# kahrendt/microWakeWord

Hardware: NVIDIA H100
Metric: streams_x_frames_per_sec (higher is better)
Workload: dtype f32

## Files before the change

### microwakeword_b200/csrc/mww_frontend.cu

```cuda
#include <cuda_runtime.h>
#include <stdlib.h>

#include "mww_frontend_dev.cuh"
#include "mww_kernels.h"

namespace mww {

__device__ __forceinline__ void cp_async16(void *smem_dst, const void *gmem_src) {
    const unsigned dst = (unsigned)__cvta_generic_to_shared(smem_dst);
    asm volatile("cp.async.cg.shared.global [%0], [%1], 16;" ::"r"(dst), "l"(gmem_src));
}
__device__ __forceinline__ void cp_async_commit_and_wait_all() {
    asm volatile("cp.async.commit_group;\ncp.async.wait_group 0;" ::: "memory");
}

__device__ __forceinline__ void k1_load_audio_async(int tid, K1Smem &sm, int buf, const int16_t *carry, int used,
                                                    const int16_t *audio, int n_samples, int f0) {
    const int base = kHop * f0;
    for (int v = tid; v < kGroupSamples / 8; v += kK1Threads) {
        const int vi = base + 8 * v;
        int16_t *dst = &sm.audio[buf][8 * v];
        if (vi < used) cp_async16(dst, carry + vi);
        else if (vi - used < n_samples) cp_async16(dst, audio + (vi - used));
        else *reinterpret_cast<uint4 *>(dst) = make_uint4(0, 0, 0, 0);
    }
}

__device__ __forceinline__ void k1_packed_load_audio_async(int tid, K1Smem &sm, const int16_t *carry, int used, const int16_t *audio,
                                                           long long audio_stride, int n_samples, long long s0, int n_streams, int spc, int fps) {
    const int span8 = (fps + 2) * (kHop / 8), used8 = used / 8, n8 = n_samples / 8;
    int16_t *dst0 = &sm.audio[0][0];
    for (int i = tid; i < spc * span8; i += kK1Threads) {
        const int sl = i / span8, v8 = i - sl * span8;
        int16_t *dst = dst0 + 8 * i;
        const long long s = s0 + sl;
        if (s < n_streams && v8 < used8) cp_async16(dst, carry + s * kWindow + 8 * v8);
        else if (s < n_streams && v8 - used8 < n8) cp_async16(dst, audio + s * audio_stride + 8 * (v8 - used8));
        else *reinterpret_cast<uint4 *>(dst) = make_uint4(0, 0, 0, 0);
    }
}

template <bool kFuseK2, int kOcc>
__global__ void __launch_bounds__(kK1Threads, kOcc)
k1_spectral_kernel(FrontendParams P, const int16_t *__restrict__ carry, int used,
                   const int16_t *__restrict__ audio, long long audio_stride, int n_samples, int n_frames,
                   int groups_per_block, int vec_ok, uint32_t *__restrict__ vout, uint32_t *__restrict__ estimate,
                   uint16_t *__restrict__ feat, long long feat_stream_stride) {
    extern __shared__ __align__(16) unsigned char k1_smem_raw[];
    K1Smem &sm = *reinterpret_cast<K1Smem *>(k1_smem_raw);
    const int tid = threadIdx.x;
    const long long s = blockIdx.x;
    K1Lane lane;
    if (kOcc <= 3) k1_lane_init(tid, P, lane);
    else k1_stage_lane_twiddles(tid, sm, P);
    const K1LaneShared lane_sh{&sm.lane_tw[tid & 15][0]};
    k1_stage_tables(tid, sm, P);

    const int n_groups = (n_frames + kFramesPerGroup - 1) / kFramesPerGroup;
    const int g_begin = blockIdx.y * groups_per_block;
    const int g_end = min(g_begin + groups_per_block, n_groups);
    const int16_t *my_carry = carry + s * kWindow;
    const int16_t *my_audio = audio + s * audio_stride;
    uint32_t est = 0;
    if (kFuseK2 && tid < kNumChannels) est = estimate[s * kNumChannels + tid];
    if (g_begin < g_end) {
        if (vec_ok) k1_load_audio_async(tid, sm, 0, my_carry, used, my_audio, n_samples, g_begin * kFramesPerGroup);
        else k1_load_audio(tid, sm, 0, my_carry, used, my_audio, n_samples, g_begin * kFramesPerGroup);
    }
    for (int g = g_begin; g < g_end; ++g) {
        const int buf = (g - g_begin) & 1;
        cp_async_commit_and_wait_all();
        __syncthreads();
        if (g + 1 < g_end) {
            if (vec_ok) k1_load_audio_async(tid, sm, buf ^ 1, my_carry, used, my_audio, n_samples, (g + 1) * kFramesPerGroup);
            else k1_load_audio(tid, sm, buf ^ 1, my_carry, used, my_audio, n_samples, (g + 1) * kFramesPerGroup);
        }
        const int f0 = g * kFramesPerGroup;
        K1Pass1Ctx ctx;
        k1_window_fft1<2>(tid, sm, buf, (kHop / 2) * (tid >> 4), P, ctx);
        __syncthreads();
        if (kOcc <= 3) k1_fft_pass2(tid, sm, lane); else k1_fft_pass2(tid, sm, lane_sh);
        __syncthreads();
        k1_real_energy(tid, sm, P);
        __syncthreads();
        const int f = f0 + (tid >> 4);
        if (!kFuseK2) {
            k1_filterbank(tid, sm, P, f < n_frames ? vout + (s * n_frames + f) * kNumChannels : nullptr);
        } else {
            k1_filterbank(tid, sm, P, &sm.A[tid >> 4][0]);
            __syncthreads();
            const int n_valid = min(kFramesPerGroup, n_frames - f0);
            if (tid < kNumChannels) k2_group_chain(tid, sm, n_valid, est);
            __syncthreads();
            k2_group_outputs(tid, sm, n_valid, feat + s * feat_stream_stride + (long long)f0 * kNumChannels);
        }
    }
    if (kFuseK2 && tid < kNumChannels) estimate[s * kNumChannels + tid] = est;
}

__global__ void __launch_bounds__(kK1Threads, 3)
k1_spectral_hop_kernel(FrontendParams P, const int16_t *__restrict__ carry, int used, const int16_t *__restrict__ audio,
                       long long audio_stride, int n_samples, int n_frames, int hop, uint32_t *__restrict__ estimate,
                       uint16_t *__restrict__ feat, long long feat_stream_stride) {
    extern __shared__ __align__(16) unsigned char k1_smem_raw[];
    K1Smem &sm = *reinterpret_cast<K1Smem *>(k1_smem_raw);
    const int tid = threadIdx.x;
    const long long s = blockIdx.x;
    K1Lane lane;
    k1_lane_init(tid, P, lane);
    k1_stage_tables(tid, sm, P);
    const int fpg = k1_hop_frames_per_group(hop);
    const int n_groups = (n_frames + fpg - 1) / fpg;
    const int16_t *my_carry = carry + s * kWindow;
    const int16_t *my_audio = audio + s * audio_stride;
    uint32_t est = 0;
    if (tid < kNumChannels) est = estimate[s * kNumChannels + tid];
    for (int g = 0; g < n_groups; ++g) {
        const int f0 = g * fpg;
        __syncthreads();
        k1_hop_load_audio(tid, sm, my_carry, used, my_audio, n_samples, hop * f0, (fpg - 1) * hop + kWindow);
        __syncthreads();
        K1Pass1Ctx ctx;
        k1_window_fft1<2>(tid, sm, 0, k1_hop_pair_base(tid >> 4, hop, fpg), P, ctx);
        __syncthreads();
        k1_fft_pass2(tid, sm, lane);
        __syncthreads();
        k1_real_energy(tid, sm, P);
        __syncthreads();
        k1_filterbank(tid, sm, P, &sm.A[tid >> 4][0]);
        __syncthreads();
        const int n_valid = min(fpg, n_frames - f0);
        if (tid < kNumChannels) k2_group_chain(tid, sm, n_valid, est);
        __syncthreads();
        k2_group_outputs(tid, sm, n_valid, feat + s * feat_stream_stride + (long long)f0 * kNumChannels);
    }
    if (tid < kNumChannels) estimate[s * kNumChannels + tid] = est;
}

__global__ void __launch_bounds__(kK1Threads, 3)
k1_spectral_packed_kernel(FrontendParams P, const int16_t *__restrict__ carry, int used,
                          const int16_t *__restrict__ audio, long long audio_stride, int n_samples, int n_streams, int fps, int spc,
                          int vec_ok, uint32_t *__restrict__ vout) {
    extern __shared__ __align__(16) unsigned char k1_smem_raw[];
    K1Smem &sm = *reinterpret_cast<K1Smem *>(k1_smem_raw);
    const int tid = threadIdx.x;
    const long long s0 = (long long)blockIdx.x * spc;
    K1Lane lane;
    k1_lane_init(tid, P, lane);
    k1_stage_tables(tid, sm, P);
    if (vec_ok) {
        k1_packed_load_audio_async(tid, sm, carry, used, audio, audio_stride, n_samples, s0, n_streams, spc, fps);
        cp_async_commit_and_wait_all();
    } else {
        k1_packed_load_audio(tid, sm, carry, used, audio, audio_stride, n_samples, s0, n_streams, spc, fps);
    }
    __syncthreads();
    const int fl = tid >> 4;
    K1Pass1Ctx ctx;
    k1_window_fft1<2>(tid, sm, 0, k1_packed_pair_base(fl < spc * fps ? fl : 0, fps), P, ctx);
    __syncthreads();
    k1_fft_pass2(tid, sm, lane);
    __syncthreads();
    k1_real_energy(tid, sm, P);
    __syncthreads();
    const long long s = s0 + fl / fps;
    const bool active = fl < spc * fps && s < n_streams;
    k1_filterbank(tid, sm, P, active ? vout + (s * fps + fl % fps) * kNumChannels : nullptr);
}

__global__ void __launch_bounds__(kK1Threads, 3)
k1k2_packed_kernel(FrontendParams P, int16_t *__restrict__ carry, int used, const int16_t *__restrict__ audio,
                   long long audio_stride, int n_samples, int n_streams, int fps, int spc, int vec_ok, uint32_t *__restrict__ estimate,
                   uint16_t *__restrict__ feat, long long feat_stream_stride, int new_used) {
    extern __shared__ __align__(16) unsigned char k1_smem_raw[];
    K1Smem &sm = *reinterpret_cast<K1Smem *>(k1_smem_raw);
    const int tid = threadIdx.x;
    const long long s0 = (long long)blockIdx.x * spc;
    K1Lane lane;
    k1_lane_init(tid, P, lane);
    k1_stage_tables(tid, sm, P);
    if (vec_ok) {
        k1_packed_load_audio_async(tid, sm, carry, used, audio, audio_stride, n_samples, s0, n_streams, spc, fps);
        cp_async_commit_and_wait_all();
    } else {
        k1_packed_load_audio(tid, sm, carry, used, audio, audio_stride, n_samples, s0, n_streams, spc, fps);
    }
    __syncthreads();
    const int fl = tid >> 4;
    K1Pass1Ctx ctx;
    k1_window_fft1<2>(tid, sm, 0, k1_packed_pair_base(fl < spc * fps ? fl : 0, fps), P, ctx);
    __syncthreads();
    k1_fft_pass2(tid, sm, lane);
    __syncthreads();
    k1_real_energy(tid, sm, P);
    __syncthreads();
    k1_filterbank(tid, sm, P, fl < spc * fps ? &sm.A[fl][0] : nullptr);
    __syncthreads();
    for (int t = tid; t < spc * kNumChannels; t += kK1Threads) {
        const int sl = t / kNumChannels, ch = t - sl * kNumChannels;
        const long long s = s0 + sl;
        if (s < n_streams) {
            const uint32_t smoothing = (ch & 1) ? kOddSmoothing : kEvenSmoothing;
            uint32_t est = estimate[s * kNumChannels + ch];
            uint16_t *out = feat + s * feat_stream_stride + ch;
            for (int f = 0; f < fps; ++f) out[(long long)f * kNumChannels] = k2_channel_step(sm.A[sl * fps + f][ch], est, smoothing, sm.gain_lut, sm.log_lut);
            estimate[s * kNumChannels + ch] = est;
        }
    }
    const int span = (fps + 2) * kHop, consumed = fps * kHop;
    const int16_t *staged = &sm.audio[0][0];
    if (vec_ok) {
        for (int i = tid; i < spc * (kWindow / 8); i += kK1Threads) {
            const int sl = i / (kWindow / 8), v8 = i - sl * (kWindow / 8);
            if (s0 + sl >= n_streams) continue;
            uint4 v = make_uint4(0, 0, 0, 0);
            if (8 * v8 < new_used) v = *reinterpret_cast<const uint4 *>(staged + sl * span + consumed + 8 * v8);
            *reinterpret_cast<uint4 *>(carry + (s0 + sl) * kWindow + 8 * v8) = v;
        }
    } else {
        for (int i = tid; i < spc * kWindow; i += kK1Threads) {
            const int sl = i / kWindow, k = i - sl * kWindow;
            if (s0 + sl >= n_streams) continue;
            carry[(s0 + sl) * kWindow + k] = k < new_used ? staged[sl * span + consumed + k] : (int16_t)0;
        }
    }
}

__global__ void __launch_bounds__(256)
k2_temporal_kernel(FrontendParams P, const uint32_t *__restrict__ vin, int n_streams, int n_frames,
                   uint32_t *__restrict__ estimate, uint16_t *__restrict__ feat, long long feat_stream_stride) {
    __shared__ int16_t gain_lut[128];
    __shared__ uint16_t log_lut[132];
    for (int i = threadIdx.x; i < 128; i += blockDim.x) gain_lut[i] = P.gain_lut[i];
    for (int i = threadIdx.x; i < 132; i += blockDim.x) log_lut[i] = P.log_lut[i];
    __syncthreads();
    const long long idx = (long long)blockIdx.x * blockDim.x + threadIdx.x;
    if (idx >= (long long)n_streams * kNumChannels) return;
    const long long s = idx / kNumChannels;
    const int ch = (int)(idx - s * kNumChannels);
    const uint32_t smoothing = (ch & 1) ? kOddSmoothing : kEvenSmoothing;
    uint32_t est = estimate[idx];
    const uint32_t *v = vin + s * (long long)n_frames * kNumChannels + ch;
    uint16_t *out = feat + s * feat_stream_stride + ch;
    int f = 0;
    for (; f + 4 <= n_frames; f += 4) {
        uint32_t x[4];
#pragma unroll
        for (int q = 0; q < 4; ++q) x[q] = __ldcs(v + (long long)(f + q) * kNumChannels);
#pragma unroll
        for (int q = 0; q < 4; ++q) out[(long long)(f + q) * kNumChannels] = k2_channel_step(x[q], est, smoothing, gain_lut, log_lut);
    }
    for (; f < n_frames; ++f) out[(long long)f * kNumChannels] = k2_channel_step(v[(long long)f * kNumChannels], est, smoothing, gain_lut, log_lut);
    estimate[idx] = est;
}

__global__ void __launch_bounds__(128)
carry_update_kernel(int16_t *__restrict__ carry, int used, const int16_t *__restrict__ audio, long long audio_stride,
                    int n_samples, int consumed, int new_used) {
    const long long s = blockIdx.x;
    int16_t *c = carry + s * kWindow;
    const int16_t *a = audio + s * audio_stride;
    int16_t tmp[4];
#pragma unroll
    for (int q = 0; q < 4; ++q) {
        const int i = threadIdx.x + 128 * q;
        int16_t val = 0;
        if (i < new_used) {
            const int vi = consumed + i;
            val = vi < used ? c[vi] : a[vi - used];
        }
        tmp[q] = val;
    }
    __syncthreads();
#pragma unroll
    for (int q = 0; q < 4; ++q) {
        const int i = threadIdx.x + 128 * q;
        if (i < kWindow) c[i] = tmp[q];
    }
}


namespace {
template <typename K>
cudaError_t k1_opt_in(K kernel, bool (&done)[64]) {
    if (!first_launch_on_this_device(done)) return cudaSuccess;
    return cudaFuncSetAttribute(kernel, cudaFuncAttributeMaxDynamicSharedMemorySize, kK1SmemBytes);
}
}

bool frontend_clip_fuses(int n_streams, int n_frames, int sm_count) {
    return n_frames > 8 && (long long)n_streams >= (long long)sm_count * 3 * 4;
}

cudaError_t launch_k1(const FrontendParams &P, const int16_t *carry, int used, const int16_t *audio,
                      long long audio_stride, int n_samples, int n_streams, int n_frames, uint32_t *vout, int sm_count,
                      cudaStream_t st) {
    if (n_frames <= 0 || n_streams <= 0) return cudaSuccess;
    const int vec_ok = (used % 8 == 0) && (n_samples % 8 == 0) && (audio_stride % 8 == 0) &&
                       (reinterpret_cast<uintptr_t>(audio) % 16 == 0) && (reinterpret_cast<uintptr_t>(carry) % 16 == 0);
    if (n_frames <= 8 && n_streams >= 2) {
        static bool done[64] = {};
        cudaError_t e = k1_opt_in(k1_spectral_packed_kernel, done);
        if (e != cudaSuccess) return e;
        const int spc = k1_packed_streams(n_frames);
        const unsigned grid = (unsigned)((n_streams + spc - 1) / spc);
        k1_spectral_packed_kernel<<<grid, kK1Threads, kK1SmemBytes, st>>>(P, carry, used, audio, audio_stride, n_samples, n_streams, n_frames, spc, vec_ok, vout);
        return cudaGetLastError();
    }
    static bool done[64] = {};
    cudaError_t e = k1_opt_in(k1_spectral_kernel<false, 3>, done);
    if (e != cudaSuccess) return e;
    const int n_groups = (n_frames + kFramesPerGroup - 1) / kFramesPerGroup;
    int chunks = 1;
    const long long want = (long long)sm_count * 3 * 4;
    if (n_streams < want) chunks = (int)min((long long)n_groups, (want + n_streams - 1) / n_streams);
    const int gpb = (n_groups + chunks - 1) / chunks;
    chunks = (n_groups + gpb - 1) / gpb;
    dim3 grid((unsigned)n_streams, (unsigned)chunks);
    k1_spectral_kernel<false, 3><<<grid, kK1Threads, kK1SmemBytes, st>>>(P, carry, used, audio, audio_stride, n_samples, n_frames, gpb, vec_ok, vout,
                                                                      nullptr, nullptr, 0);
    return cudaGetLastError();
}

cudaError_t launch_frontend_clip_fused(const FrontendParams &P, const int16_t *carry, int used, const int16_t *audio, long long audio_stride,
                                       int n_samples, int n_streams, int n_frames, uint32_t *estimate, uint16_t *feat, long long feat_stream_stride,
                                       cudaStream_t st) {
    if (n_frames <= 0 || n_streams <= 0) return cudaSuccess;
    static bool done3[64] = {}, done4[64] = {};
    static const int occ = getenv("MWW_K1_OCC") ? atoi(getenv("MWW_K1_OCC")) : 4;
    cudaError_t e = occ == 3 ? k1_opt_in(k1_spectral_kernel<true, 3>, done3) : k1_opt_in(k1_spectral_kernel<true, 4>, done4);
    if (e != cudaSuccess) return e;
    const int vec_ok = (used % 8 == 0) && (n_samples % 8 == 0) && (audio_stride % 8 == 0) &&
                       (reinterpret_cast<uintptr_t>(audio) % 16 == 0) && (reinterpret_cast<uintptr_t>(carry) % 16 == 0);
    const int n_groups = (n_frames + kFramesPerGroup - 1) / kFramesPerGroup;
    dim3 grid((unsigned)n_streams, 1u);
    if (occ == 3)
        k1_spectral_kernel<true, 3><<<grid, kK1Threads, kK1SmemBytes, st>>>(P, carry, used, audio, audio_stride, n_samples, n_frames, n_groups, vec_ok,
                                                                            nullptr, estimate, feat, feat_stream_stride);
    else
        k1_spectral_kernel<true, 4><<<grid, kK1Threads, kK1SmemBytes, st>>>(P, carry, used, audio, audio_stride, n_samples, n_frames, n_groups, vec_ok,
                                                                            nullptr, estimate, feat, feat_stream_stride);
    return cudaGetLastError();
}

cudaError_t launch_frontend_hop(const FrontendParams &P, const int16_t *carry, int used, const int16_t *audio, long long audio_stride,
                                int n_samples, int n_streams, int n_frames, int hop, uint32_t *estimate, uint16_t *feat,
                                long long feat_stream_stride, cudaStream_t st) {
    if (n_frames <= 0 || n_streams <= 0) return cudaSuccess;
    static bool done[64] = {};
    cudaError_t e = k1_opt_in(k1_spectral_hop_kernel, done);
    if (e != cudaSuccess) return e;
    k1_spectral_hop_kernel<<<(unsigned)n_streams, kK1Threads, kK1SmemBytes, st>>>(P, carry, used, audio, audio_stride, n_samples, n_frames, hop,
                                                                                 estimate, feat, feat_stream_stride);
    return cudaGetLastError();
}

bool frontend_fusable(int used, int n_samples, int n_frames) {
    const int new_used = used + n_samples - n_frames * kHop;
    return n_frames >= 1 && n_frames <= 8 && new_used >= 0 && new_used <= 2 * kHop;
}

cudaError_t launch_frontend_fused(const FrontendParams &P, int16_t *carry, int used, const int16_t *audio,
                                  long long audio_stride, int n_samples, int n_streams, int n_frames, uint32_t *estimate, uint16_t *feat,
                                  long long feat_stream_stride, cudaStream_t st) {
    if (n_streams <= 0) return cudaSuccess;
    static bool done[64] = {};
    cudaError_t e = k1_opt_in(k1k2_packed_kernel, done);
    if (e != cudaSuccess) return e;
    const int vec_ok = (used % 8 == 0) && (n_samples % 8 == 0) && (audio_stride % 8 == 0) &&
                       (reinterpret_cast<uintptr_t>(audio) % 16 == 0) && (reinterpret_cast<uintptr_t>(carry) % 16 == 0);
    const int spc = k1_packed_streams(n_frames);
    const unsigned grid = (unsigned)((n_streams + spc - 1) / spc);
    k1k2_packed_kernel<<<grid, kK1Threads, kK1SmemBytes, st>>>(P, carry, used, audio, audio_stride, n_samples, n_streams, n_frames, spc, vec_ok,
                                                    estimate, feat, feat_stream_stride, used + n_samples - n_frames * kHop);
    return cudaGetLastError();
}

cudaError_t launch_k2(const FrontendParams &P, const uint32_t *vin, int n_streams, int n_frames, uint32_t *estimate,
                      uint16_t *feat, long long feat_stream_stride, cudaStream_t st) {
    if (n_frames <= 0 || n_streams <= 0) return cudaSuccess;
    const long long total = (long long)n_streams * kNumChannels;
    const unsigned blocks = (unsigned)((total + 255) / 256);
    k2_temporal_kernel<<<blocks, 256, 0, st>>>(P, vin, n_streams, n_frames, estimate, feat, feat_stream_stride);
    return cudaGetLastError();
}

cudaError_t launch_carry_update(int16_t *carry, int used, const int16_t *audio, long long audio_stride, int n_samples,
                                int n_streams, int consumed, int new_used, cudaStream_t st) {
    if (n_streams <= 0) return cudaSuccess;
    carry_update_kernel<<<(unsigned)n_streams, 128, 0, st>>>(carry, used, audio, audio_stride, n_samples, consumed, new_used);
    return cudaGetLastError();
}

}
```

### microwakeword_b200/csrc/mww_frontend_dev.cuh

```cuda
#pragma once

#include "mww_common.h"
#include "mww_tables.h"

#if !defined(__CUDA_ARCH__)
#include <math.h>
#endif

namespace mww {

constexpr int kFramesPerGroup = 16;
constexpr int kK1Threads = 256;
constexpr int kRowWords = 272;
constexpr int kGroupSamples = (kFramesPerGroup + 2) * kHop;


struct K1Smem {
    uint32_t A[kFramesPerGroup][kRowWords];
    uint32_t B[kFramesPerGroup][kRowWords];
    int16_t audio[2][kGroupSamples];
    uint16_t lane_max[kFramesPerGroup][16];
    int32_t shift[kFramesPerGroup];
    int32_t fb_coef[kFbCoefWords];
    int16_t gain_lut[128];
    uint16_t log_lut[132];
    uint32_t lane_tw[16][15];
};
constexpr int kK1SmemBytes = (int)sizeof(K1Smem);

MWW_HD void k1_stage_tables(int tid, K1Smem &sm, const FrontendParams &P) {
    for (int i = tid; i < kFbCoefWords; i += kK1Threads) sm.fb_coef[i] = P.fb_coef[i];
    for (int i = tid; i < 128; i += kK1Threads) sm.gain_lut[i] = P.gain_lut[i];
    for (int i = tid; i < 132; i += kK1Threads) sm.log_lut[i] = P.log_lut[i];
}

struct K1Lane {
    int32_t t3r[3], t3i[3];
    int32_t t4r[12], t4i[12];
};

struct K1LaneShared { const uint32_t *row; };


MWW_HD int32_t fixdiv4(int32_t x) { return (x * 8191 + 16384) >> 15; }
MWW_HD int32_t fixdiv2(int32_t x) { return (x * 16383 + 16384) >> 15; }

MWW_HD void cmul_q15(int32_t ar, int32_t ai, int32_t wr, int32_t wi, int32_t &mr, int32_t &mi) {
    mr = (ar * wr - ai * wi + 16384) >> 15;
    mi = (ar * wi + ai * wr + 16384) >> 15;
}

MWW_HD void bfly4_core(int32_t &r0, int32_t &i0, int32_t &r1, int32_t &i1, int32_t &r2, int32_t &i2, int32_t &r3, int32_t &i3) {
    const int32_t s5r = r0 - r2, s5i = i0 - i2;
    const int32_t f0r = r0 + r2, f0i = i0 + i2;
    const int32_t s3r = r1 + r3, s3i = i1 + i3;
    const int32_t s4r = r1 - r3, s4i = i1 - i3;
    r2 = f0r - s3r; i2 = f0i - s3i;
    r0 = f0r + s3r; i0 = f0i + s3i;
    r1 = s5r + s4i; i1 = s5i - s4r;
    r3 = s5r - s4i; i3 = s5i + s4r;
}


MWW_HD uint64_t sq32(uint32_t r) { return (uint64_t)r * r; }

MWW_HD uint32_t isqrt64_round(uint64_t x) {
#if defined(__CUDA_ARCH__)
    const float xf = __ull2float_rn(x);
    const float rs = rsqrtf(xf);
    uint32_t r = __float2uint_rz(xf * rs);
    const int64_t d = (int64_t)(x - sq32(r));
    const int64_t r1 = (int64_t)r + (int64_t)__float2int_rd(__ll2float_rn(d) * (0.5f * rs));
#else
    const float xf = (float)x;
    const float rs = x ? 1.0f / sqrtf(xf) : 0.0f;
    const float rf = xf * rs;
    uint32_t r = rf >= 4294967040.0f ? 0xFFFFFFFFu : (uint32_t)rf;
    const int64_t d = (int64_t)(x - sq32(r));
    const int64_t r1 = (int64_t)r + (int64_t)floorf((float)d * (0.5f * rs));
#endif
    r = r1 > 0xFFFFFFFFll ? 0xFFFFFFFFu : (r1 < 0 ? 0u : (uint32_t)r1);
#pragma unroll
    for (int pass = 0; pass < 2; ++pass) r -= (sq32(r) > x) ? 1u : 0u;
    uint64_t rem = x - sq32(r);
#pragma unroll
    for (int pass = 0; pass < 2; ++pass) {
        const bool up = rem > 2ull * r;
        rem -= up ? 2ull * r + 1 : 0ull;
        r += up ? 1u : 0u;
    }
    const uint32_t cap = (x >> 32) == 0 ? 0xFFFFu : 0xFFFFFFFFu;
    r += (rem > r && r < cap) ? 1u : 0u;
    r = r > cap ? cap : r;
    return x == 0 ? 0u : r;
}

MWW_HD uint32_t isqrt64_round_fast(uint64_t x) {
    if (x >> 48) return isqrt64_round(x);
#if defined(__CUDA_ARCH__)
    const uint32_t r = __double2uint_rz(sqrt(__ull2double_rn(x)) + 0.5);
#else
    const uint32_t r = (uint32_t)(sqrt((double)x) + 0.5);
#endif
    const uint32_t cap = (x >> 32) == 0 ? 0xFFFFu : 0xFFFFFFFFu;
    return r > cap ? cap : r;
}


MWW_HD void k1_lane_init(int tid, const FrontendParams &P, K1Lane &L) {
    const int b = tid & 15;
    for (int j = 0; j < 3; ++j) {
        const uint32_t w = P.tw[4 * b * (j + 1)];
        L.t3r[j] = unpack_lo(w); L.t3i[j] = unpack_hi(w);
    }
    for (int j = 0; j < 4; ++j) {
        const int kp = 16 * j + b;
        for (int q = 0; q < 3; ++q) {
            const uint32_t w = P.tw[kp * (q + 1)];
            L.t4r[3 * j + q] = unpack_lo(w); L.t4i[3 * j + q] = unpack_hi(w);
        }
    }
}

MWW_HD void k1_stage_lane_twiddles(int tid, K1Smem &sm, const FrontendParams &P) {
    for (int i = tid; i < 16 * 15; i += kK1Threads) {
        const int b = i / 15, e = i - 15 * b;
        int idx;
        if (e < 3) idx = 4 * b * (e + 1);
        else { const int j = (e - 3) / 3, q = (e - 3) - 3 * j; idx = (16 * j + b) * (q + 1); }
        sm.lane_tw[b][e] = P.tw[idx];
    }
}
MWW_HD void lane_tw3(const K1Lane &L, int q, int32_t &wr, int32_t &wi) { wr = L.t3r[q]; wi = L.t3i[q]; }
MWW_HD void lane_tw4(const K1Lane &L, int i, int32_t &wr, int32_t &wi) { wr = L.t4r[i]; wi = L.t4i[i]; }
MWW_HD void lane_tw3(const K1LaneShared &L, int q, int32_t &wr, int32_t &wi) { const uint32_t w = L.row[q]; wr = unpack_lo(w); wi = unpack_hi(w); }
MWW_HD void lane_tw4(const K1LaneShared &L, int i, int32_t &wr, int32_t &wi) { const uint32_t w = L.row[3 + i]; wr = unpack_lo(w); wi = unpack_hi(w); }

MWW_HD void k1_load_audio(int tid, K1Smem &sm, int buf, const int16_t *carry, int used, const int16_t *audio, int n_samples, int f0) {
    const int base = kHop * f0;
    for (int i = tid; i < kGroupSamples; i += kK1Threads) {
        const int vi = base + i;
        int16_t s = 0;
        if (vi < used) s = carry[vi];
        else if (vi - used < n_samples) s = audio[vi - used];
        sm.audio[buf][i] = s;
    }
}

MWW_HD int k1_hop_frames_per_group(int hop) {
    const int by_span = (2 * kGroupSamples - kWindow) / hop + 1;
    return by_span < kFramesPerGroup ? by_span : kFramesPerGroup;
}
MWW_HD void k1_hop_load_audio(int tid, K1Smem &sm, const int16_t *carry, int used, const int16_t *audio, int n_samples, int base, int span) {
    int16_t *dst = &sm.audio[0][0];
    for (int i = tid; i < span; i += kK1Threads) {
        const int vi = base + i;
        int16_t s = 0;
        if (vi < used) s = carry[vi];
        else if (vi - used < n_samples) s = audio[vi - used];
        dst[i] = s;
    }
}
MWW_HD int k1_hop_pair_base(int fl, int hop, int fpg) { return (hop / 2) * (fl < fpg ? fl : fpg - 1); }

struct K1Pass1Ctx { int32_t xr[16], xi[16]; };

template <int PART>
MWW_HD void k1_window_fft1(int tid, K1Smem &sm, int buf, int pair_base, const FrontendParams &P, K1Pass1Ctx &ctx) {
    const int fl = tid >> 4, a = tid & 15;
    const int c = (a >> 2) + 4 * (a & 3);
    int32_t (&xr)[16] = ctx.xr;
    int32_t (&xi)[16] = ctx.xi;
    if (PART != 1) {
        const uint32_t *pairs = reinterpret_cast<const uint32_t *>(sm.audio[buf]) + pair_base;
        int32_t mx = 0, mn = 0;
#pragma unroll
        for (int b = 0; b < 16; ++b) {
            const int j = (b >> 2) + 4 * (b & 3);
            if (j == 15) { xr[b] = 0; xi[b] = 0; continue; }
            const int p = c + 16 * j;
            const uint32_t sw = pairs[p];
            const uint32_t cw = P.win_pairs[p];
            const int32_t v0 = (unpack_lo(sw) * unpack_lo(cw)) >> 12;
            const int32_t v1 = (unpack_hi(sw) * unpack_hi(cw)) >> 12;
            xr[b] = v0; xi[b] = v1;
            if (j == 7) {
                const int32_t m0 = v0 == -32768 ? 0 : v0, m1 = v1 == -32768 ? 0 : v1;
                mx = max3i(mx, m0, m1); mn = min3i(mn, m0, m1);
            } else {
                mx = max3i(mx, v0, v1); mn = min3i(mn, v0, v1);
            }
        }
        const int32_t m = mx > -mn ? mx : -mn;
        sm.lane_max[fl][a] = (uint16_t)m;
    }
#if defined(__CUDA_ARCH__)
    if (PART == 2) __syncwarp();
#endif
    if (PART == 0) return;
    int32_t mxa = 0;
#pragma unroll
    for (int i = 0; i < 16; ++i) { const int32_t v = sm.lane_max[fl][i]; mxa = v > mxa ? v : mxa; }
    const int shift = 15 - msb32((uint32_t)mxa);
    if (a == 0) sm.shift[fl] = shift;
    const int32_t k4 = 8191 << shift;
#pragma unroll
    for (int g = 0; g < 4; ++g) {
#pragma unroll
        for (int q = 0; q < 4; ++q) {
            const int b = 4 * g + q;
            const int j = (b >> 2) + 4 * (b & 3);
            if (j == 7) {
                xr[b] = fixdiv4(sext16(xr[b] << shift)); xi[b] = fixdiv4(sext16(xi[b] << shift));
            } else {
                xr[b] = (xr[b] * k4 + 16384) >> 15; xi[b] = (xi[b] * k4 + 16384) >> 15;
            }
        }
        bfly4_core(xr[4 * g], xi[4 * g], xr[4 * g + 1], xi[4 * g + 1], xr[4 * g + 2], xi[4 * g + 2], xr[4 * g + 3], xi[4 * g + 3]);
    }
#pragma unroll
    for (int k = 0; k < 4; ++k) {
#pragma unroll
        for (int q = 0; q < 4; ++q) { xr[k + 4 * q] = fixdiv4(xr[k + 4 * q]); xi[k + 4 * q] = fixdiv4(xi[k + 4 * q]); }
        if (k > 0) {
#pragma unroll
            for (int q = 1; q < 4; ++q) {
                int32_t mr, mi;
                cmul_q15(xr[k + 4 * q], xi[k + 4 * q], P.tw2[(k - 1) * 3 + (q - 1)][0], P.tw2[(k - 1) * 3 + (q - 1)][1], mr, mi);
                xr[k + 4 * q] = mr; xi[k + 4 * q] = mi;
            }
        }
        bfly4_core(xr[k], xi[k], xr[k + 4], xi[k + 4], xr[k + 8], xi[k + 8], xr[k + 12], xi[k + 12]);
    }
#pragma unroll
    for (int b = 0; b < 16; ++b) sm.B[fl][17 * a + b] = pack16(xr[b], xi[b]);
}

MWW_HD int k1_packed_streams(int fps) {
    const int by_slots = kFramesPerGroup / fps;
    const int by_smem = (2 * kGroupSamples) / ((fps + 2) * kHop);
    return by_slots < by_smem ? by_slots : by_smem;
}
MWW_HD void k1_packed_load_audio(int tid, K1Smem &sm, const int16_t *carry, int used, const int16_t *audio, long long audio_stride,
                                 int n_samples, long long s0, int n_streams, int spc, int fps) {
    const int span = (fps + 2) * kHop;
    int16_t *dst = &sm.audio[0][0];
    for (int i = tid; i < spc * span; i += kK1Threads) {
        const int sl = i / span, vi = i - sl * span;
        int16_t v = 0;
        if (s0 + sl < n_streams) {
            if (vi < used) v = carry[(s0 + sl) * kWindow + vi];
            else if (vi - used < n_samples) v = audio[(s0 + sl) * audio_stride + (vi - used)];
        }
        dst[i] = v;
    }
}
MWW_HD int k1_packed_pair_base(int fl, int fps) { return (fl / fps) * ((fps + 2) * (kHop / 2)) + (kHop / 2) * (fl % fps); }

template <typename LaneT>
MWW_HD void k1_fft_pass2(int tid, K1Smem &sm, const LaneT &L) {
    const int fl = tid >> 4, b = tid & 15;
    int32_t yr[16], yi[16];
#pragma unroll
    for (int a = 0; a < 16; ++a) {
        const uint32_t w = sm.B[fl][17 * a + b];
        yr[a] = unpack_lo(w); yi[a] = unpack_hi(w);
    }
#pragma unroll
    for (int c = 0; c < 4; ++c) {
#pragma unroll
        for (int q = 0; q < 4; ++q) { yr[4 * c + q] = fixdiv4(yr[4 * c + q]); yi[4 * c + q] = fixdiv4(yi[4 * c + q]); }
#pragma unroll
        for (int q = 1; q < 4; ++q) {
            int32_t mr, mi, wr, wi;
            lane_tw3(L, q - 1, wr, wi);
            cmul_q15(yr[4 * c + q], yi[4 * c + q], wr, wi, mr, mi);
            yr[4 * c + q] = mr; yi[4 * c + q] = mi;
        }
        bfly4_core(yr[4 * c], yi[4 * c], yr[4 * c + 1], yi[4 * c + 1], yr[4 * c + 2], yi[4 * c + 2], yr[4 * c + 3], yi[4 * c + 3]);
    }
#pragma unroll
    for (int j = 0; j < 4; ++j) {
#pragma unroll
        for (int q = 0; q < 4; ++q) { yr[4 * q + j] = fixdiv4(sext16(yr[4 * q + j])); yi[4 * q + j] = fixdiv4(sext16(yi[4 * q + j])); }
#pragma unroll
        for (int q = 1; q < 4; ++q) {
            int32_t mr, mi, wr, wi;
            lane_tw4(L, 3 * j + q - 1, wr, wi);
            cmul_q15(yr[4 * q + j], yi[4 * q + j], wr, wi, mr, mi);
            yr[4 * q + j] = mr; yi[4 * q + j] = mi;
        }
        bfly4_core(yr[j], yi[j], yr[4 + j], yi[4 + j], yr[8 + j], yi[8 + j], yr[12 + j], yi[12 + j]);
    }
#pragma unroll
    for (int a = 0; a < 16; ++a) sm.A[fl][b + 16 * a] = pack16(yr[a], yi[a]);
}

MWW_HD void k1_real_energy(int tid, K1Smem &sm, const FrontendParams &P) {
    const int fl = tid >> 4, l = tid & 15;
    if (l == 0) { sm.B[fl][0] = 0; sm.B[fl][kEnergyOffset] = 0; }
#pragma unroll
    for (int t = 0; t < 8; ++t) {
        const int k = 1 + 16 * t + l;
        const uint32_t wk = sm.A[fl][k];
        const uint32_t wn = sm.A[fl][kNcfft - k];
        const uint32_t ws = P.super_tw[k - 1];
        const int32_t pr = fixdiv2(unpack_lo(wk)), pi = fixdiv2(unpack_hi(wk));
        const int32_t nr = fixdiv2(unpack_lo(wn)), ni = fixdiv2(sext16(-unpack_hi(wn)));
        const int32_t f1r = pr + nr, f1i = pi + ni;
        const int32_t f2r = pr - nr, f2i = pi - ni;
        int32_t tr, ti;
        cmul_q15(f2r, f2i, unpack_lo(ws), unpack_hi(ws), tr, ti);
        tr = sext16(tr); ti = sext16(ti);
        const int32_t ar = sext16((f1r + tr) >> 1), ai = sext16((f1i + ti) >> 1);
        const int32_t br = sext16((f1r - tr) >> 1), bi = sext16((ti - f1i) >> 1);
        sm.B[fl][k + kEnergyOffset] = (uint32_t)(ar * ar) + (uint32_t)(ai * ai);
        sm.B[fl][kNcfft - k + kEnergyOffset] = (uint32_t)(br * br) + (uint32_t)(bi * bi);
    }
}

struct Pair32 { uint32_t x, y; };
MWW_HD Pair32 load_pair(const uint32_t *p) {
#if defined(__CUDA_ARCH__)
    const uint2 v = *reinterpret_cast<const uint2 *>(p);
    return Pair32{v.x, v.y};
#else
    return Pair32{p[0], p[1]};
#endif
}
MWW_HD void k1_filterbank(int tid, K1Smem &sm, const FrontendParams &P, uint32_t *vout_frame ) {
    const int fl = tid >> 4, l = tid & 15;
    const int sh = sm.shift[fl];
#pragma unroll
    for (int s = 0; s < kFbSlots; ++s) {
        if (fb_len(s) == 0) continue;
        const FbSlot slot = P.fb_slots[l * kFbSlots + s];
        int64_t acc = 0;
        const uint32_t *e = &sm.B[fl][slot.word0];
        const uint32_t *cf = reinterpret_cast<const uint32_t *>(&sm.fb_coef[slot.coef_off]);
#pragma unroll
        for (int j = 0; j < fb_len(s) / 2; ++j) {
            const Pair32 ev = load_pair(e + 2 * j), cv = load_pair(cf + 2 * j);
            acc = mad_wide_s32((int32_t)ev.x, (int32_t)cv.x, acc);
            acc = mad_wide_s32((int32_t)ev.y, (int32_t)cv.y, acc);
        }
        if (slot.ch >= 0 && vout_frame) vout_frame[slot.ch] = isqrt64_round_fast((uint64_t)acc) >> sh;
    }
}


MWW_HD int32_t wide_dynamic_function(uint32_t x, const int16_t *lut) {
    if (x <= 2) return lut[x];
    const int interval = msb32(x);
    const int16_t *p = lut + 4 * interval - 6;
    const int32_t frac = (int32_t)(((interval < 11) ? (x << (11 - interval)) : (x >> (interval - 11))) & 0x3FF);
    int32_t r = ((int32_t)p[2] * frac) >> 5;
    r += (int32_t)((uint32_t)(int32_t)p[1] << 5);
    r *= frac;
    r = (r + (1 << 14)) >> 15;
    r += p[0];
    return (int32_t)(int16_t)r;
}

MWW_HD uint32_t pcan_shrink(uint32_t x) {
    if (x < (2u << 12)) return (x * x) >> 20;
    return (x >> 6) - 64u;
}

MWW_HD uint32_t log_scale(uint32_t x, const uint16_t *lut) {
    const uint32_t integer = (uint32_t)msb32(x) - 1;
    int32_t frac = (int32_t)(x - (1u << integer));
    if (integer < 16) frac <<= (16 - integer); else frac >>= (integer - 16);
    const uint32_t seg = (uint32_t)frac >> 9;
    const int32_t c0 = lut[seg], c1 = lut[seg + 1];
    const int32_t rel = ((c1 - c0) * (frac - (int32_t)(seg << 9))) >> 16;
    const uint32_t log2v = (integer << 16) + (uint32_t)(frac + c0 + rel);
    const uint32_t loge = (uint32_t)((45426ull * log2v + 32768u) >> 16);
    return ((loge << kLogScaleShift) + 32768u) >> 16;
}

MWW_HD uint32_t k2_estimate_update(uint32_t v, uint32_t est, uint32_t smoothing) {
    const uint32_t scaled = v << kSmoothingBits;
    return (uint32_t)((((uint64_t)scaled * smoothing) + ((uint64_t)est * ((1u << kNoiseBits) - smoothing))) >> kNoiseBits);
}

MWW_HD uint16_t k2_output(uint32_t v, uint32_t est, const int16_t *gain_lut, const uint16_t *log_lut) {
    const uint32_t scaled = v << kSmoothingBits;
    const uint32_t e = est > scaled ? scaled : est;
    const uint32_t fl = (uint32_t)(((uint64_t)v * kMinSignalRemaining) >> kNoiseBits);
    const uint32_t sub = (scaled - e) >> kSmoothingBits;
    uint32_t sig = sub > fl ? sub : fl;
    const uint32_t gain = (uint32_t)wide_dynamic_function(est, gain_lut);
    const uint32_t snr = (uint32_t)(((uint64_t)sig * gain) >> kPcanSnrShift);
    sig = pcan_shrink(snr);
    sig <<= kLogCorrectionBits;
    sig = sig > 1 ? log_scale(sig, log_lut) : 0;
    return (uint16_t)(sig < 0xFFFFu ? sig : 0xFFFFu);
}

MWW_HD uint16_t k2_channel_step(uint32_t v, uint32_t &est, uint32_t smoothing, const int16_t *gain_lut, const uint16_t *log_lut) {
    est = k2_estimate_update(v, est, smoothing);
    return k2_output(v, est, gain_lut, log_lut);
}

MWW_HD void k2_group_chain(int ch, K1Smem &sm, int n_valid, uint32_t &est) {
    const uint32_t smoothing = (ch & 1) ? kOddSmoothing : kEvenSmoothing;
    for (int f = 0; f < n_valid; ++f) {
        est = k2_estimate_update(sm.A[f][ch], est, smoothing);
        sm.B[f][ch] = est;
    }
}
MWW_HD void k2_group_outputs(int tid, K1Smem &sm, int n_valid, uint16_t *feat_group ) {
    for (int i = tid; i < n_valid * kNumChannels; i += kK1Threads) {
        const int f = i / kNumChannels, ch = i - f * kNumChannels;
        feat_group[i] = k2_output(sm.A[f][ch], sm.B[f][ch], sm.gain_lut, sm.log_lut);
    }
}

}
```

Before: 460.9 million.

## Stage twiddles in padded smem, shuffle-reduce lane max, defer wide isqrt path

```diff
diff --git a/microwakeword_b200/csrc/mww_frontend.cu b/microwakeword_b200/csrc/mww_frontend.cu
--- a/microwakeword_b200/csrc/mww_frontend.cu
+++ b/microwakeword_b200/csrc/mww_frontend.cu
@@ -10,6 +10,10 @@
     const unsigned dst = (unsigned)__cvta_generic_to_shared(smem_dst);
     asm volatile("cp.async.cg.shared.global [%0], [%1], 16;" ::"r"(dst), "l"(gmem_src));
 }
+__device__ __forceinline__ void cp_async16_zfill(void *smem_dst, const void *gmem_src, bool valid) {
+    const unsigned dst = (unsigned)__cvta_generic_to_shared(smem_dst);
+    asm volatile("cp.async.cg.shared.global [%0], [%1], 16, %2;" ::"r"(dst), "l"(gmem_src), "r"(valid ? 16 : 0));
+}
 __device__ __forceinline__ void cp_async_commit_and_wait_all() {
     asm volatile("cp.async.commit_group;\ncp.async.wait_group 0;" ::: "memory");
 }
@@ -17,12 +21,11 @@
 __device__ __forceinline__ void k1_load_audio_async(int tid, K1Smem &sm, int buf, const int16_t *carry, int used,
                                                     const int16_t *audio, int n_samples, int f0) {
     const int base = kHop * f0;
+#pragma unroll 1
     for (int v = tid; v < kGroupSamples / 8; v += kK1Threads) {
         const int vi = base + 8 * v;
-        int16_t *dst = &sm.audio[buf][8 * v];
-        if (vi < used) cp_async16(dst, carry + vi);
-        else if (vi - used < n_samples) cp_async16(dst, audio + (vi - used));
-        else *reinterpret_cast<uint4 *>(dst) = make_uint4(0, 0, 0, 0);
+        const bool from_carry = vi < used, valid = from_carry || vi - used < n_samples;
+        cp_async16_zfill(&sm.audio[buf][8 * v], from_carry || !valid ? carry + (from_carry ? vi : 0) : audio + (vi - used), valid);
     }
 }
 
diff --git a/microwakeword_b200/csrc/mww_frontend_dev.cuh b/microwakeword_b200/csrc/mww_frontend_dev.cuh
--- a/microwakeword_b200/csrc/mww_frontend_dev.cuh
+++ b/microwakeword_b200/csrc/mww_frontend_dev.cuh
@@ -24,7 +24,8 @@
     int32_t fb_coef[kFbCoefWords];
     int16_t gain_lut[128];
     uint16_t log_lut[132];
-    uint32_t lane_tw[16][15];
+    alignas(16) uint32_t lane_tw[16][15 * 4];
+    alignas(16) int32_t super_tw[128][4];
 };
 constexpr int kK1SmemBytes = (int)sizeof(K1Smem);
 
@@ -32,7 +33,12 @@
     for (int i = tid; i < kFbCoefWords; i += kK1Threads) sm.fb_coef[i] = P.fb_coef[i];
     for (int i = tid; i < 128; i += kK1Threads) sm.gain_lut[i] = P.gain_lut[i];
     for (int i = tid; i < 132; i += kK1Threads) sm.log_lut[i] = P.log_lut[i];
-}
+    for (int i = tid; i < 128; i += kK1Threads) {
+        const uint32_t w = P.super_tw[i];
+        sm.super_tw[i][0] = unpack_lo(w); sm.super_tw[i][1] = unpack_hi(w); sm.super_tw[i][2] = -unpack_hi(w); sm.super_tw[i][3] = 0;
+    }
+}
+static_assert(4 * (sizeof(K1Smem) + 1024) <= 228 * 1024, "K1Smem must leave room for 4 CTAs per SM");
 
 struct K1Lane {
     int32_t t3r[3], t3i[3];
@@ -47,6 +53,10 @@
 
 MWW_HD void cmul_q15(int32_t ar, int32_t ai, int32_t wr, int32_t wi, int32_t &mr, int32_t &mi) {
     mr = (ar * wr - ai * wi + 16384) >> 15;
+    mi = (ar * wi + ai * wr + 16384) >> 15;
+}
+MWW_HD void cmul_q15_nw(int32_t ar, int32_t ai, int32_t wr, int32_t wi, int32_t nwi, int32_t &mr, int32_t &mi) {
+    mr = (ar * wr + ai * nwi + 16384) >> 15;
     mi = (ar * wi + ai * wr + 16384) >> 15;
 }
 
@@ -95,16 +105,17 @@
     return x == 0 ? 0u : r;
 }
 
-MWW_HD uint32_t isqrt64_round_fast(uint64_t x) {
-    if (x >> 48) return isqrt64_round(x);
+MWW_HD uint32_t isqrt64_round_fp64(uint64_t x) {
 #if defined(__CUDA_ARCH__)
     const uint32_t r = __double2uint_rz(sqrt(__ull2double_rn(x)) + 0.5);
 #else
-    const uint32_t r = (uint32_t)(sqrt((double)x) + 0.5);
+    const double s = sqrt((double)x) + 0.5;
+    const uint32_t r = s >= 4294967296.0 ? 0xFFFFFFFFu : (uint32_t)s;
 #endif
     const uint32_t cap = (x >> 32) == 0 ? 0xFFFFu : 0xFFFFFFFFu;
     return r > cap ? cap : r;
 }
+MWW_HD uint32_t isqrt64_round_fast(uint64_t x) { return (x >> 48) ? isqrt64_round(x) : isqrt64_round_fp64(x); }
 
 
 MWW_HD void k1_lane_init(int tid, const FrontendParams &P, K1Lane &L) {
@@ -128,13 +139,24 @@
         int idx;
         if (e < 3) idx = 4 * b * (e + 1);
         else { const int j = (e - 3) / 3, q = (e - 3) - 3 * j; idx = (16 * j + b) * (q + 1); }
-        sm.lane_tw[b][e] = P.tw[idx];
-    }
-}
-MWW_HD void lane_tw3(const K1Lane &L, int q, int32_t &wr, int32_t &wi) { wr = L.t3r[q]; wi = L.t3i[q]; }
-MWW_HD void lane_tw4(const K1Lane &L, int i, int32_t &wr, int32_t &wi) { wr = L.t4r[i]; wi = L.t4i[i]; }
-MWW_HD void lane_tw3(const K1LaneShared &L, int q, int32_t &wr, int32_t &wi) { const uint32_t w = L.row[q]; wr = unpack_lo(w); wi = unpack_hi(w); }
-MWW_HD void lane_tw4(const K1LaneShared &L, int i, int32_t &wr, int32_t &wi) { const uint32_t w = L.row[3 + i]; wr = unpack_lo(w); wi = unpack_hi(w); }
+        const uint32_t w = P.tw[idx];
+        uint32_t *q = &sm.lane_tw[b][4 * e];
+        q[0] = (uint32_t)unpack_lo(w); q[1] = (uint32_t)unpack_hi(w); q[2] = (uint32_t)-unpack_hi(w); q[3] = 0;
+    }
+}
+MWW_HD void lane_tw(const K1Lane &L, int e, int32_t &wr, int32_t &wi, int32_t &nwi) {
+    wr = e < 3 ? L.t3r[e] : L.t4r[e - 3]; wi = e < 3 ? L.t3i[e] : L.t4i[e - 3]; nwi = -wi;
+}
+MWW_HD void load_tw(const void *entry, int32_t &wr, int32_t &wi, int32_t &nwi) {
+#if defined(__CUDA_ARCH__)
+    const int4 v = *reinterpret_cast<const int4 *>(entry);
+    wr = v.x; wi = v.y; nwi = v.z;
+#else
+    const int32_t *p = reinterpret_cast<const int32_t *>(entry);
+    wr = p[0]; wi = p[1]; nwi = p[2];
+#endif
+}
+MWW_HD void lane_tw(const K1LaneShared &L, int e, int32_t &wr, int32_t &wi, int32_t &nwi) { load_tw(L.row + 4 * e, wr, wi, nwi); }
 
 MWW_HD void k1_load_audio(int tid, K1Smem &sm, int buf, const int16_t *carry, int used, const int16_t *audio, int n_samples, int f0) {
     const int base = kHop * f0;
@@ -171,6 +193,7 @@
     const int c = (a >> 2) + 4 * (a & 3);
     int32_t (&xr)[16] = ctx.xr;
     int32_t (&xi)[16] = ctx.xi;
+    int32_t m = 0;
     if (PART != 1) {
         const uint32_t *pairs = reinterpret_cast<const uint32_t *>(sm.audio[buf]) + pair_base;
         int32_t mx = 0, mn = 0;
@@ -191,16 +214,19 @@
                 mx = max3i(mx, v0, v1); mn = min3i(mn, v0, v1);
             }
         }
-        const int32_t m = mx > -mn ? mx : -mn;
-        sm.lane_max[fl][a] = (uint16_t)m;
-    }
-#if defined(__CUDA_ARCH__)
-    if (PART == 2) __syncwarp();
-#endif
+        m = mx > -mn ? mx : -mn;
+        if (PART == 0) sm.lane_max[fl][a] = (uint16_t)m;
+    }
     if (PART == 0) return;
     int32_t mxa = 0;
+#if defined(__CUDA_ARCH__)
+    mxa = m;
+#pragma unroll
+    for (int o = 8; o > 0; o >>= 1) { const int32_t v = __shfl_xor_sync(0xFFFFFFFFu, mxa, o); mxa = v > mxa ? v : mxa; }
+#else
 #pragma unroll
     for (int i = 0; i < 16; ++i) { const int32_t v = sm.lane_max[fl][i]; mxa = v > mxa ? v : mxa; }
+#endif
     const int shift = 15 - msb32((uint32_t)mxa);
     if (a == 0) sm.shift[fl] = shift;
     const int32_t k4 = 8191 << shift;
@@ -272,9 +298,9 @@
         for (int q = 0; q < 4; ++q) { yr[4 * c + q] = fixdiv4(yr[4 * c + q]); yi[4 * c + q] = fixdiv4(yi[4 * c + q]); }
 #pragma unroll
         for (int q = 1; q < 4; ++q) {
-            int32_t mr, mi, wr, wi;
-            lane_tw3(L, q - 1, wr, wi);
-            cmul_q15(yr[4 * c + q], yi[4 * c + q], wr, wi, mr, mi);
+            int32_t mr, mi, wr, wi, nwi;
+            lane_tw(L, q - 1, wr, wi, nwi);
+            cmul_q15_nw(yr[4 * c + q], yi[4 * c + q], wr, wi, nwi, mr, mi);
             yr[4 * c + q] = mr; yi[4 * c + q] = mi;
         }
         bfly4_core(yr[4 * c], yi[4 * c], yr[4 * c + 1], yi[4 * c + 1], yr[4 * c + 2], yi[4 * c + 2], yr[4 * c + 3], yi[4 * c + 3]);
@@ -285,9 +311,9 @@
         for (int q = 0; q < 4; ++q) { yr[4 * q + j] = fixdiv4(sext16(yr[4 * q + j])); yi[4 * q + j] = fixdiv4(sext16(yi[4 * q + j])); }
 #pragma unroll
         for (int q = 1; q < 4; ++q) {
-            int32_t mr, mi, wr, wi;
-            lane_tw4(L, 3 * j + q - 1, wr, wi);
-            cmul_q15(yr[4 * q + j], yi[4 * q + j], wr, wi, mr, mi);
+            int32_t mr, mi, wr, wi, nwi;
+            lane_tw(L, 3 + 3 * j + q - 1, wr, wi, nwi);
+            cmul_q15_nw(yr[4 * q + j], yi[4 * q + j], wr, wi, nwi, mr, mi);
             yr[4 * q + j] = mr; yi[4 * q + j] = mi;
         }
         bfly4_core(yr[j], yi[j], yr[4 + j], yi[4 + j], yr[8 + j], yi[8 + j], yr[12 + j], yi[12 + j]);
@@ -296,7 +322,7 @@
     for (int a = 0; a < 16; ++a) sm.A[fl][b + 16 * a] = pack16(yr[a], yi[a]);
 }
 
-MWW_HD void k1_real_energy(int tid, K1Smem &sm, const FrontendParams &P) {
+MWW_HD void k1_real_energy(int tid, K1Smem &sm, const FrontendParams &) {
     const int fl = tid >> 4, l = tid & 15;
     if (l == 0) { sm.B[fl][0] = 0; sm.B[fl][kEnergyOffset] = 0; }
 #pragma unroll
@@ -304,13 +330,14 @@
         const int k = 1 + 16 * t + l;
         const uint32_t wk = sm.A[fl][k];
         const uint32_t wn = sm.A[fl][kNcfft - k];
-        const uint32_t ws = P.super_tw[k - 1];
+        int32_t wr, wi, nwi;
+        load_tw(sm.super_tw[k - 1], wr, wi, nwi);
         const int32_t pr = fixdiv2(unpack_lo(wk)), pi = fixdiv2(unpack_hi(wk));
         const int32_t nr = fixdiv2(unpack_lo(wn)), ni = fixdiv2(sext16(-unpack_hi(wn)));
         const int32_t f1r = pr + nr, f1i = pi + ni;
         const int32_t f2r = pr - nr, f2i = pi - ni;
         int32_t tr, ti;
-        cmul_q15(f2r, f2i, unpack_lo(ws), unpack_hi(ws), tr, ti);
+        cmul_q15_nw(f2r, f2i, wr, wi, nwi, tr, ti);
         tr = sext16(tr); ti = sext16(ti);
         const int32_t ar = sext16((f1r + tr) >> 1), ai = sext16((f1i + ti) >> 1);
         const int32_t br = sext16((f1r - tr) >> 1), bi = sext16((ti - f1i) >> 1);
@@ -328,23 +355,40 @@
     return Pair32{p[0], p[1]};
 #endif
 }
+MWW_HD uint64_t fb_accumulate(const uint32_t *e, const uint32_t *cf, int len ) {
+    int64_t acc = 0;
+#pragma unroll
+    for (int j = 0; j < len / 2; ++j) {
+        const Pair32 ev = load_pair(e + 2 * j), cv = load_pair(cf + 2 * j);
+        acc = mad_wide_s32((int32_t)ev.x, (int32_t)cv.x, acc);
+        acc = mad_wide_s32((int32_t)ev.y, (int32_t)cv.y, acc);
+    }
+    return (uint64_t)acc;
+}
 MWW_HD void k1_filterbank(int tid, K1Smem &sm, const FrontendParams &P, uint32_t *vout_frame ) {
     const int fl = tid >> 4, l = tid & 15;
     const int sh = sm.shift[fl];
+    bool wide = false;
 #pragma unroll
     for (int s = 0; s < kFbSlots; ++s) {
         if (fb_len(s) == 0) continue;
         const FbSlot slot = P.fb_slots[l * kFbSlots + s];
-        int64_t acc = 0;
-        const uint32_t *e = &sm.B[fl][slot.word0];
-        const uint32_t *cf = reinterpret_cast<const uint32_t *>(&sm.fb_coef[slot.coef_off]);
-#pragma unroll
-        for (int j = 0; j < fb_len(s) / 2; ++j) {
-            const Pair32 ev = load_pair(e + 2 * j), cv = load_pair(cf + 2 * j);
-            acc = mad_wide_s32((int32_t)ev.x, (int32_t)cv.x, acc);
-            acc = mad_wide_s32((int32_t)ev.y, (int32_t)cv.y, acc);
-        }
-        if (slot.ch >= 0 && vout_frame) vout_frame[slot.ch] = isqrt64_round_fast((uint64_t)acc) >> sh;
+        const uint64_t x = fb_accumulate(&sm.B[fl][slot.word0], reinterpret_cast<const uint32_t *>(&sm.fb_coef[slot.coef_off]), fb_len(s));
+        wide |= (x >> 48) != 0;
+        if (slot.ch >= 0 && vout_frame) vout_frame[slot.ch] = isqrt64_round_fp64(x) >> sh;
+    }
+    if (wide && vout_frame) {
+#pragma unroll 1
+        for (int s = 0; s < kFbSlots; ++s) {
+            const FbSlot slot = P.fb_slots[l * kFbSlots + s];
+            if (fb_len(s) == 0 || slot.ch < 0) continue;
+            const uint32_t *e = &sm.B[fl][slot.word0];
+            const int32_t *cf = &sm.fb_coef[slot.coef_off];
+            int64_t acc = 0;
+#pragma unroll 1
+            for (int j = 0; j < fb_len(s); ++j) acc = mad_wide_s32((int32_t)e[j], cf[j], acc);
+            if ((uint64_t)acc >> 48) vout_frame[slot.ch] = isqrt64_round((uint64_t)acc) >> sh;
+        }
     }
 }
 
```

New measurement: 474.4 million, median of 6. 1.03x the previous value.
